# cmaestre/pcl_tracking

Measured on AMD Instinct MI355X. Metric: particles x input-points / sec per frame (tracked frames/sec @8192 particles per GPU), higher is better.
Workload: dtype f32

## Files before the change

### pcl_tracking_amd/csrc/pft_api.hip

```cpp
#include <math.h>
#include <stdio.h>
#include <string.h>

#include <stdlib.h>

#include <algorithm>
#include <cmath>
#include <string>
#include <vector>

#include "pft_internal.h"
#include "../../include/pft_segment.h"

#define HIPCHK(t, call)                                                                       \
  do {                                                                                        \
    hipError_t e_ = (call);                                                                   \
    if (e_ != hipSuccess) {                                                                   \
      (t)->err = std::string(#call) + ": " + hipGetErrorString(e_);                           \
      return PFT_ERR_HIP;                                                                     \
    }                                                                                         \
  } while (0)

struct EvPair {
  hipEvent_t a, b;
// ... 508 lines not shown
  if (debug) {
    HIPCHK(t, dalloc(&n.b.mark, cap));
    HIPCHK(t, dalloc(&n.pts, cap));
  }
  n.b.cap = cap;
  n.b.tab_cap = tab;
  if (c.b.st) {
    HIPCHK(t, hipMemcpyAsync(n.b.st, c.b.st, sizeof(PftChangeState), hipMemcpyDeviceToDevice, t->stream));
    for (int k = 0; k < 2; k++) {
      HIPCHK(t, hipMemcpyAsync(n.b.set_key[k], c.b.set_key[k], (size_t)c.b.cap * 8u, hipMemcpyDeviceToDevice, t->stream));
      HIPCHK(t, hipMemcpyAsync(n.b.set_cnt[k], c.b.set_cnt[k], (size_t)c.b.cap * 4u, hipMemcpyDeviceToDevice, t->stream));
    }
    HIPCHK(t, hipStreamSynchronize(t->stream));
  } else {
    HIPCHK(t, hipMemsetAsync(n.b.st, 0, sizeof(PftChangeState), t->stream));
  }
  cd_free(c);
  c = n;
  return PFT_OK;
}

PftSwitches pft_read_switches() {
  auto on = [](const char* name) { return getenv(name) != nullptr; };
  auto is1 = [](const char* name) { const char* e = getenv(name); return e && e[0] == '1'; };
  PftSwitches w = {};
  w.graph = is1("PFT_GRAPH");
  if (const char* b = getenv("PFT_FORCE_BUILDER")) w.builder = !strcmp(b, "single") ? 1 : (!strcmp(b, "sorted") ? 2 : 0);
  w.leaf_indirect = on("PFT_LEAF_INDIRECT") ? (int)is1("PFT_LEAF_INDIRECT") : -1;
  w.aabb_full = on("PFT_AABB_FULL");
  w.resample_one_lane = on("PFT_RESAMPLE_ONE_LANE");
  w.split_resample = on("PFT_SPLIT_RESAMPLE") || w.resample_one_lane;
  w.crop_two_pass = on("PFT_CROP_TWO_PASS");
  w.generic_descent = is1("PFT_GENERIC_DESCENT");
  w.ancestor_table = !on("PFT_ANCESTOR_TABLE") || is1("PFT_ANCESTOR_TABLE");
  w.exact_path = on("PFT_EXACT_SHELLS_ONLY") ? PftExactPath::shells : on("PFT_EXACT_PER_QUERY") ? PftExactPath::per_query : PftExactPath::sorted;
#ifdef PFT_DIAG
  if (const char* a = getenv("PFT_ABLATE")) w.ablate = atoi(a);
  w.skip_octree = on("PFT_DEBUG_SKIP_OCTREE");
#endif
  return w;
}

#ifdef PFT_DIAG
extern "C" void pft_debug_set_ablate(pft_tracker* t, int mask) { if (t) t->sw.ablate = mask; }
#endif

extern "C" int pft_create(const pft_config* cfg, pft_tracker** out) {
  if (!cfg || !out) return PFT_ERR_INVALID_ARG;
  *out = nullptr;
  if (cfg->abi_version != PFT_ABI_VERSION || cfg->particle_num <= 0 || cfg->iteration_num <= 0 ||
      cfg->world_size <= 0 || cfg->rank < 0 || cfg->rank >= cfg->world_size || cfg->use_normal != 0 ||
      cfg->particle_num % cfg->world_size != 0 || !(cfg->octree_resolution > 0) ||
      (cfg->sum_order != PFT_SUM_TREE && cfg->sum_order != PFT_SUM_PCL))
    return PFT_ERR_INVALID_ARG;
  if (cfg->particle_num > PFT_MAX_PARTICLES) return PFT_ERR_CAPACITY;
  if (cfg->kld_adaptive) {
    if (cfg->world_size != 1 || cfg->maximum_particle_num <= 0 || !(cfg->kld_epsilon > 0)) return PFT_ERR_INVALID_ARG;
    for (int k = 0; k < 6; k++)
      if (!(cfg->kld_bin_size[k] > 0)) return PFT_ERR_INVALID_ARG;
    if (cfg->maximum_particle_num >= PFT_POPM_MIN || cfg->particle_num >= PFT_POPM_MIN) return PFT_ERR_CAPACITY;
  }
  int ndev = 0;
  if (hipGetDeviceCount(&ndev) != hipSuccess || ndev <= 0 || cfg->device_id >= ndev) return PFT_ERR_NO_DEVICE;
  if (hipSetDevice(cfg->device_id) != hipSuccess) return PFT_ERR_NO_DEVICE;
  hipDeviceProp_t prop;
  if (hipGetDeviceProperties(&prop, cfg->device_id) != hipSuccess) return PFT_ERR_NO_DEVICE;

// ... 59 lines not shown
  A(dalloc(&t->d_jump, (size_t)1 << (3 * PFT_JUMP_MAX_LEVEL)));
  if (t->sw.ancestor_table) A(dalloc(&t->d_anc, PFT_ANC_CAP));
  A(dalloc(&t->d_alias_list, 2 * Pt));
  A(dalloc(&t->d_alias_pref, 2 * Pt));
  A(dalloc(&t->d_pop_part, (size_t)PFT_POPM_MAX_WGS * 16));
  A(dalloc(&t->d_alias_pos, Pt));
  A(dalloc(&t->d_raw_w, Pt));
  if (cfg->exact_nearest) {
    A(dalloc(&t->d_eg_start, (size_t)PFT_EG_CAP + 1));
    A(dalloc(&t->d_eg_cnt, (size_t)PFT_EG_CAP));
    A(dalloc(&t->d_eg_tile, (size_t)PFT_EG_CAP / 2048 + 2));
    A(dalloc(&t->d_ec_slot, (size_t)PFT_EG_CAP));
    A(dalloc(&t->d_ec_cells, (size_t)PFT_EC_SLOTS));
    A(dalloc(&t->d_ec_count, (size_t)PFT_EC_SLOTS));
    A(dalloc(&t->d_ec_base, (size_t)PFT_EC_SLOTS));
    t->ec_pool_cap = PFT_EC_POOL_MIN;
    A(dalloc(&t->d_ec_list, (size_t)t->ec_pool_cap));
    A(dalloc(&t->d_eq_cellq, (size_t)PFT_EG_CAP));
    A(dalloc(&t->d_eq_nq, (size_t)PFT_EC_SLOTS));
    A(dalloc(&t->d_eq_qbase, (size_t)PFT_EC_SLOTS));
    A(dalloc(&t->d_eq_bbase, (size_t)PFT_EC_SLOTS));
    A(dalloc(&t->d_eq_fill, (size_t)PFT_EC_SLOTS));
  }
  if (p.kld) {
    A(dalloc(&t->d_kld_table, (size_t)6 * p.kld_max + 128));
    A(dalloc(&t->d_kld_bins, (size_t)6 * p.kld_max));
  }
  A(hipHostMalloc(reinterpret_cast<void**>(&t->h_stat), 8 * sizeof(uint32_t), hipHostMallocMapped));
  if (t->h_stat) for (int i = 0; i < 8; i++) t->h_stat[i] = 0;
  A(dalloc(&t->d_hdr, 1));
  A(dalloc(&t->d_dbg_hdr, 1));
  if (e == hipSuccess) e = hipMemsetAsync(t->d_hdr, 0, sizeof(PftHeader), t->stream);
  if (e == hipSuccess) e = hipMemsetAsync(t->d_dbg_hdr, 0, sizeof(PftHeader), t->stream);
  if (e != hipSuccess) {
    pft_destroy(t);
    return PFT_ERR_HIP;
  }
  if (cfg->max_input_points) {
    int r = ensure_input_capacity(t, cfg->max_input_points);
    if (r != PFT_OK) {
      pft_destroy(t);
      return r;
    }
  }
  sync_dev(t);
  *out = t;
  return PFT_OK;
}

static void release_borrow(pft_tracker* t) {
  PftBorrow* b = t->borrow;
  t->borrow = nullptr;
  if (!b) return;
  b->tracker_alive = false;
  b->armed = false;
  if (!b->filter_alive) {
    hipEventDestroy(b->ev);
    delete b;
  }
}

extern "C" void pft_destroy(pft_tracker* t) {
  if (!t) return;
  if (t->stream) hipStreamSynchronize(t->stream);
  release_borrow(t);
  dfree(t->d_n_in);
// ... 2049 lines not shown
```

### pcl_tracking_amd/csrc/pft_device_utils.h

```cpp
#pragma once
#include <float.h>
#include <math.h>

#include "pft_internal.h"

#define WAVE 64
#define UNROLL_FENCE(j, every) do { if (((j) % (every)) == (every) - 1) __builtin_amdgcn_sched_barrier(0); } while (0)

__device__ __forceinline__ bool pft_unchanged(const uint32_t* gate) { return gate && *gate == 0u; }

__device__ __forceinline__ int lane_id() { return threadIdx.x & (WAVE - 1); }
__device__ __forceinline__ int wave_id() { return threadIdx.x >> 6; }

template <typename T>
__device__ __forceinline__ T wave_sum(T v) {
#pragma unroll
  for (int o = 32; o > 0; o >>= 1) v += __shfl_xor(v, o);
  return v;
}
template <int CTRL, int ROW_MASK>
__device__ __forceinline__ double dpp_move_f64(double v) {
  const unsigned long long b = (unsigned long long)__double_as_longlong(v);
  const int lo = __builtin_amdgcn_update_dpp(0, (int)(uint32_t)b, CTRL, ROW_MASK, 0xf, false);
  const int hi = __builtin_amdgcn_update_dpp(0, (int)(uint32_t)(b >> 32), CTRL, ROW_MASK, 0xf, false);
// ... 161 lines not shown
  float A = (float)cos((double)q.yaw), B = (float)sin((double)q.yaw);
  float C = (float)cos((double)q.pitch), D = (float)sin((double)q.pitch);
  float E = (float)cos((double)q.roll), F = (float)sin((double)q.roll);
  float DE = D * E, DF = D * F;
  m[0] = A * C;  m[1] = A * DF - B * E;  m[2] = B * F + A * DE;  m[3] = q.x;
  m[4] = B * C;  m[5] = A * E + B * DF;  m[6] = B * DE - A * F;  m[7] = q.y;
  m[8] = -D;     m[9] = C * F;           m[10] = C * E;          m[11] = q.z;
}

__device__ __forceinline__ void store_matrix(float* mats, uint32_t i, const float* m) {
  float4* dst = reinterpret_cast<float4*>(mats + 12 * (size_t)i);
  dst[0] = make_float4(m[0], m[1], m[2], m[3]);
  dst[1] = make_float4(m[4], m[5], m[6], m[7]);
  dst[2] = make_float4(m[8], m[9], m[10], m[11]);
}

__device__ __forceinline__ void load_matrix(const float* mats, uint32_t i, float* T) {
  const float4* tp = reinterpret_cast<const float4*>(mats + 12 * (size_t)i);
  float4 r0 = tp[0], r1 = tp[1], r2 = tp[2];
  T[0] = r0.x; T[1] = r0.y; T[2] = r0.z; T[3] = r0.w;
  T[4] = r1.x; T[5] = r1.y; T[6] = r1.z; T[7] = r1.w;
  T[8] = r2.x; T[9] = r2.y; T[10] = r2.z; T[11] = r2.w;
}

__device__ __forceinline__ void xform(const float* T, float x, float y, float z, float& ox, float& oy, float& oz) {
  ox = T[0] * x + T[1] * y + T[2] * z + T[3];
  oy = T[4] * x + T[5] * y + T[6] * z + T[7];
  oz = T[8] * x + T[9] * y + T[10] * z + T[11];
}

#include "pft_alias.h"

__device__ inline void pft_anc_window(PftHeader* hdr, const PftDev& d, int D, bool on, const double mn[3], double res) {
  const int L = D - PFT_ANC_UP;
  on = on && d.anc != nullptr && L >= 1;
  const float inv = (float)(1.0 / res);
  uint32_t lo[3] = {0u, 0u, 0u}, bits[3] = {0u, 0u, 0u};
  for (int a = 0; a < 3 && on; a++) {
    const float om = (float)mn[a];
    const float f0 = fmaxf(floorf((hdr->bbox[2 * a] - om) * inv), 0.0f);
    const float f1 = fmaxf(floorf((hdr->bbox[2 * a + 1] - om) * inv), 0.0f);
    const uint32_t top = (1u << L) - 1u;
    const uint32_t c0 = min(f0 < 2147483648.0f ? (uint32_t)f0 >> PFT_ANC_UP : top, top);
    const uint32_t c1 = min(f1 < 2147483648.0f ? (uint32_t)f1 >> PFT_ANC_UP : top, top);
    on = c1 >= c0;
    const uint32_t n = c1 - c0 + 1u;
    bits[a] = n > 1u ? 32u - (uint32_t)__clz((int)(n - 1u)) : 0u;
    lo[a] = min(c0, (1u << L) - (1u << bits[a]));
  }
  on = on && bits[0] + bits[1] + bits[2] <= PFT_ANC_CAP_BITS;
  hdr->anc_level = on ? L : 0;
  for (int a = 0; a < 3; a++) {
    hdr->anc_lo[a] = on ? lo[a] : 0u;
    hdr->anc_bits[a] = on ? bits[a] : 0u;
  }
  hdr->build_epoch = hdr->build_epoch + 1u;
}
```

### pcl_tracking_amd/csrc/pft_internal.h

```cpp
#pragma once
#include <hip/hip_runtime.h>
#include <stdint.h>

#include <vector>

#include "../../include/pft.h"

#define PFT_MAX_DEVICES 64
#define PFT_MAX_DEPTH 30
#define PFT_TABLE_MAX_DEPTH 10
#define PFT_MAX_GROW 40
#define PFT_JUMP_MAX_LEVEL 4
#ifndef PFT_ANC_CAP_BITS
#define PFT_ANC_CAP_BITS 18
#endif
#define PFT_ANC_CAP (1u << PFT_ANC_CAP_BITS)
#ifndef PFT_ANC_UP
#define PFT_ANC_UP 2
#endif
#define PFT_REF_CHUNK 256
#ifndef PFT_BUILD_THREADS
#define PFT_BUILD_THREADS 1024
#endif
#ifndef PFT_LIK_GROUPS
#define PFT_LIK_GROUPS 64
#endif
#ifndef PFT_LIK_CTR_STRIDE
#define PFT_LIK_CTR_STRIDE 16u
#endif
#ifndef PFT_LIK_THREADS
#define PFT_LIK_THREADS 1024
#endif
#ifndef PFT_LIK_WGS_PER_CU
#define PFT_LIK_WGS_PER_CU 2
#endif
#define PFT_POP_THREADS 1024
#define PFT_SORTED_BUILD_MIN 18000
#define PFT_EG_CAP (1u << 21)
#define PFT_EC_SLOTS (1u << 19)
#define PFT_EC_POOL (1u << 24)
#define PFT_EC_POOL_MIN (1u << 20)
#define PFT_POPM_THREADS 256
#define PFT_POPM_ITEMS 16
#define PFT_POPM_MAX_WGS 256
#define PFT_POPM_MIN (16 * PFT_POP_THREADS + 1)
#define PFT_MAX_PARTICLES (PFT_POPM_MAX_WGS * PFT_POPM_THREADS * PFT_POPM_ITEMS)

struct PftParams {
  double alpha;
  double maxd2;
  double res;
  double dist_w, hsv_w;
// ... 6 lines not shown
  uint32_t M_box;
  uint32_t ref_chunk;
  uint32_t split_last;
  uint32_t kld;
  uint32_t kld_max;
  double kld_z;
  double kld_eps;
  float kld_bin[6];
  double motion_ratio;
  int32_t sum_order;
};

struct PftHeader {
  float bbox[6];
  uint32_t n_crop;
  uint32_t error;
  double omin[3], omax[3];
  int32_t depth;
  int32_t use_table;
  uint32_t n_words;
  uint32_t n_leaves;
  uint32_t leaf_start;
  uint32_t lvl_start[PFT_MAX_DEPTH + 3];
  int32_t n_grow;
  int32_t build_path;
  uint32_t build_variant;
  int32_t leaf_indirect;
  int32_t jump_level;
  float margin_cells;
  float ominf[3];
  float inv_res;
  int32_t anc_level;
  uint32_t anc_lo[3], anc_bits[3];
  uint32_t build_epoch;
  uint32_t anc_epoch;
  uint32_t grow_idx[PFT_MAX_GROW];
  uint32_t grow_shift[PFT_MAX_GROW];
  uint32_t grow_old_depth[PFT_MAX_GROW];
  double grow_min[PFT_MAX_GROW + 1][3];
  double fit_ratio;
  pft_particle rep;
  pft_particle motion;
  uint32_t alias_m, alias_nh;
  float eg_g, eg_inv_g, eg_min[3];
  int32_t eg_dim[3];
  uint32_t eg_ncells;
  uint32_t p_active;
  uint32_t kld_k;
  unsigned long long stat_queries, stat_scanned;
  unsigned long long dbg[32];
  unsigned long long ticks[32];
  alignas(128) uint32_t lik_ctr[PFT_LIK_GROUPS * PFT_LIK_CTR_STRIDE];
  alignas(128) uint32_t ec_nslots;
  uint32_t ec_pool_used;
  unsigned long long eq_totals;
  alignas(128) uint32_t crop_ticket;
  uint32_t pop_bar[4];
  unsigned long long dbg_hard[5];
  uint32_t lik_layout[4];
};

struct PftDev {
  const float4* ref_xyz;
  const float4* ref_hsv;
  const float4* ref_box;
  const float4* in_pts;
// ... 101 lines not shown
  size_t n_in;
  int device_id;
  hipEvent_t done;
};
int pftf_view(pft_filter* f, PftFilterView* v);
void pftf_attach(pft_filter* f, PftBorrow* b);

void pftk_remove_zero_points(hipStream_t s, const pft_point_xyzrgba* in, uint32_t n, float4* xyz, uint8_t* flag,
                             uint32_t* tile, uint32_t* keep_idx, float4* keep_xyz, uint32_t* n_keep);
struct pft_segment;
int pftsg_device_id(const pft_segment* s);
struct pft_model;
struct PftModelView {
  const pft_point_xyzrgba* recentred;
  size_t n_recentred;
  const pft_point_xyzrgba* reference;
  size_t n_reference;
  float trans[16];
  uint32_t first_nonfinite;
  int device_id;
};
int pftm_view(const pft_model* m, PftModelView* v);

enum class PftExactPath { sorted, per_query, shells };
struct PftSwitches {
  bool graph;
  int builder;
  int leaf_indirect;
  bool aabb_full;
  bool split_resample;
  bool resample_one_lane;
  bool crop_two_pass;
  bool generic_descent;
  bool ancestor_table;
  PftExactPath exact_path;
  int ablate;
  bool skip_octree;
};
PftSwitches pft_read_switches();

void pftk_report(hipStream_t s, const pft_point_xyzrgba* pts, uint32_t n, const PftHeader* hdr, int sum_order,
                 pft_point_xyzrgba* tracked, pft_object_report* out);
void pftk_match(hipStream_t s, const PftParams& p, const PftDev& d, double min_ratio, uint32_t lost_after,
                pft_match_stats* out, int32_t* input_idx, float* sq_dist);
uint32_t pftk_spread_blocks(uint32_t n_max);
void pftk_spread(hipStream_t s, const PftDev& d, uint32_t n_max, double* part, uint32_t* part_zero, float* part_wmax,
                 uint32_t* part_imax, double max_pos_sigma, double min_n_eff, uint32_t after, pft_population_stats* out);
struct PftRqLattice {
  uint32_t n[3];
  float base[3], span[3];
};
struct PftRqScores {
  uint32_t *n_inliers, *n_matched;
  double *coherence, *sum_sq_dist, *inlier_sq_dist;
};
void pftk_reacquire_centroids(hipStream_t s, const pft_point_xyzrgba* pts, const uint32_t* first, const uint32_t* count,
                              uint32_t n_clusters, float* centres);
void pftk_reacquire_candidates(hipStream_t s, const float* centres, uint32_t K, const PftRqLattice& lat, pft_particle* part,
                               float* mats);
void pftk_reacquire_score(hipStream_t s, const PftParams& p, const PftDev& d, uint32_t K, double inlier_d2,
                          const PftRqScores& out);
void pftk_reacquire_select(hipStream_t s, const PftParams& p, const PftDev& d, const PftRqScores& sc, uint32_t K,
                           uint32_t n_centres, uint32_t per_centre, double accept_ratio, pft_reacquire_result* out);
struct PftRefineCtl;
struct PftRefineDev {
  PftRefineCtl* ctl;
  double* part;
// ... 59 lines not shown
```

### pcl_tracking_amd/csrc/pft_likelihood.hip

```cpp
#include "pft_device_utils.h"

#ifndef PFT_LIK_PENALTY
#define PFT_LIK_PENALTY 1
#endif

struct LikCtx {
  const uint32_t* words;
  const float* tab;
  uint32_t per_axis;
  const float* lut_h;
  const float* lut_s;
  const float* pen;
  const uint16_t* jump;
  int J;
  uint32_t lvlJ_start;
  const uint32_t* anc;
  uint32_t alo, abits;
  float margin, near_thr, ominx, ominy, ominz, inv_res, ncell;
  uint32_t leaf0;
  const uint16_t* leaf16;
};

struct HybridWords {
  const __attribute__((address_space(3))) uint32_t* lds;
  const uint32_t* __restrict__ glob;
  uint32_t n_lds;
  __device__ __forceinline__ uint32_t operator[](uint32_t i) const { return i < n_lds ? lds[i] : glob[i]; }
};

__device__ __forceinline__ double rcp_nr(double x) {
  double r = __builtin_amdgcn_rcp(x);
  double e = fma(-x, r, 1.0);
  r = fma(r, e, r);
  e = fma(-x, r, 1.0);
  r = fma(r, e, r);
  return r;
}

__device__ __forceinline__ bool face_violation(uint32_t kx, uint32_t ky, uint32_t kz, uint32_t lowf, uint32_t highf,
                                               int sh) {
  const uint32_t mx = (1u << sh) - 1u;
  const uint32_t rx = kx & mx, ry = ky & mx, rz = kz & mx;
  bool v = ((lowf & 1u) && rx == 0) || ((highf & 1u) && rx == mx);
  v |= ((lowf & 2u) && ry == 0) || ((highf & 2u) && ry == mx);
  v |= ((lowf & 4u) && rz == 0) || ((highf & 4u) && rz == mx);
  return v;
}

__device__ __forceinline__ int near_face_level(uint32_t k, bool low, bool high) {
  const uint32_t t = low ? k : ~k;
  const uint32_t c = min((uint32_t)(t == 0u ? -1 : __builtin_ctz(t)), 31u);
  return (low | high) ? (int)c : -1;
}

template <bool USE_TAB, bool FAST, bool DEBUG_NN, int LEAF, bool INDIRECT, typename WordPtr>
__device__ __forceinline__ void likelihood_items(const PftParams& prm, const PftDev& d, const LikCtx& cx, WordPtr W,
                                                 uint32_t n_particles, int D, uint32_t n_crop,
                                                 const double omin[3], int abl) {
  const int lane = lane_id(), w = wave_id(), nw = blockDim.x >> 6;
  const uint32_t M = prm.M, nchunk = prm.nchunk;
  const uint32_t G = min((uint32_t)PFT_LIK_GROUPS, gridDim.x), grp = blockIdx.x % G;
  const uint32_t gq = gridDim.x / G, gr = gridDim.x % G;
  const uint32_t wgs_in_grp = gq + (grp < gr ? 1u : 0u), waves_in_grp = wgs_in_grp * (uint32_t)nw;
  const uint32_t wgs_before = grp * gq + min(grp, gr);
  const uint32_t pb = (uint32_t)((unsigned long long)n_particles * wgs_before / gridDim.x);
  const uint32_t pe = (uint32_t)((unsigned long long)n_particles * (wgs_before + wgs_in_grp) / gridDim.x);
  const uint32_t np_grp = pe - pb, nbig = prm.split_last ? nchunk - prm.split_last : nchunk, nsmall = nchunk - nbig;
  const uint32_t small_len = prm.split_last ? prm.ref_chunk / prm.split_last : 0u;
  const uint32_t it_begin = 0u, it_end = np_grp * nchunk, big_items = np_grp * nbig;
  const uint32_t lw = (blockIdx.x / G) * (uint32_t)nw + (uint32_t)w;
  uint32_t* ctr = &d.hdr->lik_ctr[grp * PFT_LIK_CTR_STRIDE];
  const double res = prm.res;
  const double maxd2 = prm.maxd2;
  const double wd = prm.dist_w, whsv = prm.hsv_w;
  const float hw = prm.h_w, sw = prm.s_w, vw = prm.v_w;
  for (uint32_t item_v = it_begin + lw; item_v < it_end;) {
    const uint32_t item = (uint32_t)__builtin_amdgcn_readfirstlane((int)item_v);
    uint32_t pi, ch, cstart, clen;
    if (item < big_items) {
      pi = pb + item / nbig;
      ch = item % nbig;
      cstart = ch * prm.ref_chunk;
      clen = prm.ref_chunk;
    } else {
      const uint32_t r = item - big_items;
      pi = pb + r / nsmall;
      ch = nbig + r % nsmall;
      cstart = nbig * prm.ref_chunk + (r % nsmall) * small_len;
// ... 12 lines not shown
      float qx, qy, qz;
      xform(T, r.x, r.y, r.z, qx, qy, qz);
      if (n_crop == 0) {
        if (DEBUG_NN) {
          const size_t o = (size_t)pi * M + d.ref_perm[j];
          d.nn_idx[o] = -1;
          d.nn_d2[o] = INFINITY;
        }
        continue;
      }
      uint32_t node = 0, jx = 1, jy = 1, jz = 1;
      int lvl = 0;
      int dbg_fast = 0, dbg_gen = 0, dbg_jump = 0, dbg_hard = 0;
      if (FAST) {
        const float tx = (qx - cx.ominx) * cx.inv_res, ty = (qy - cx.ominy) * cx.inv_res,
                    tz = (qz - cx.ominz) * cx.inv_res;
        const float flx = floorf(tx), fly = floorf(ty), flz = floorf(tz);
        const bool inside = (int)(fminf(fminf(tx, ty), tz) >= 0.0f) & (int)(fmaxf(fmaxf(tx, ty), tz) < cx.ncell);
        const float fx = tx - flx, fy = ty - fly, fz = tz - flz;
        const float mg = cx.margin, mh = 1.0f - cx.margin;
        const uint32_t kx = inside ? (uint32_t)flx : 0u, ky = inside ? (uint32_t)fly : 0u,
                       kz = inside ? (uint32_t)flz : 0u;
        int V = -1;
        const float off = fmaxf(fmaxf(fabsf(fx - 0.5f), fabsf(fy - 0.5f)), fabsf(fz - 0.5f));
        if (__builtin_amdgcn_ballot_w64(off > cx.near_thr)) {
          const int vx = near_face_level(kx, fx < mg, fx > mh), vy = near_face_level(ky, fy < mg, fy > mh),
                    vz = near_face_level(kz, fz < mg, fz > mh);
          V = max(vx, max(vy, vz));
        }
        V = inside ? V : 31;
        int lim = min(D, D - 1 - V);
        bool inw = false;
        uint32_t ae = 0u;
        if (!INDIRECT && LEAF == 1 && cx.anc) {
          const uint32_t bx = cx.abits & 0xffu, by = (cx.abits >> 8) & 0xffu, bz = cx.abits >> 16;
          const uint32_t ux = (kx >> PFT_ANC_UP) - (cx.alo & 1023u), uy = (ky >> PFT_ANC_UP) - ((cx.alo >> 10) & 1023u),
                         uz = (kz >> PFT_ANC_UP) - (cx.alo >> 20);
          inw = ((ux >> bx) | (uy >> by) | (uz >> bz)) == 0u;
          ae = cx.anc[inw ? ux | (uy << bx) | (uz << (bx + by)) : 0u];
        }
        const int a = (int)(ae >> 27);
        const bool hit = inw & (a <= lim);
        node = hit ? (ae & 0x7ffffffu) : 0u;
        lvl = hit ? a : 0;
        lim = (hit & (a < D - PFT_ANC_UP)) ? a : lim;
        if (cx.J > 0 && __builtin_amdgcn_ballot_w64(!hit)) {
          const int sh = D - cx.J;
          const uint32_t e = cx.jump[(kx >> sh) | ((ky >> sh) << cx.J) | ((kz >> sh) << (2 * cx.J))];
          const bool take = !hit & (cx.J <= lim) & (e != 0u);
          node = take ? cx.lvlJ_start + e - 1u : node;
          lvl = take ? cx.J : lvl;
          if (DEBUG_NN) dbg_jump = take ? 1 : 0;
        }
        while (lvl < lim) {
          const int sh = D - lvl - 1;
          const uint32_t c = (((kx >> sh) & 1u) << 2) | (((ky >> sh) & 1u) << 1) | ((kz >> sh) & 1u);
          const uint32_t wv = W[node];
          if (!((wv >> c) & 1u)) break;
          node = (wv >> 8) + __popc(wv & 0xffu & ((1u << c) - 1u));
          lvl++;
          dbg_fast++;
        }
        const int up = D - lvl;
        const uint32_t top = 1u << lvl;
        jx = (kx >> up) | top; jy = (ky >> up) | top; jz = (kz >> up) | top;
      }
      if ((abl & 1) && lvl < D) {
        node = cx.leaf0;
        lvl = D;
      }
      for (; lvl < D; lvl++) {
        dbg_gen++;
        const uint32_t wv = W[node];
        const uint32_t mask = wv & 0xffu, base = wv >> 8;
        float cx0, cx1, cy0, cy1, cz0, cz1;
        if (USE_TAB) {
          const float2 tx2 = *reinterpret_cast<const float2*>(cx.tab - 2 + 2u * jx);
          const float2 ty2 = *reinterpret_cast<const float2*>(cx.tab + cx.per_axis - 2 + 2u * jy);
// ... 153 lines not shown
          hd2 = fabsf(1.0f + rh.x - th);
        else
          hd2 = fabsf(1.0f + th - rh.x);
        float h_diff;
        if (hd1 < hd2)
          h_diff = hw * hd1 * hd1;
        else
          h_diff = hw * hd2 * hd2;
        const float s_diff = sw * (rh.y - ts) * (rh.y - ts);
        const float v_diff = vw * (rh.z - tv) * (rh.z - tv);
        const float diff2 = h_diff + s_diff + v_diff;
        double Bq = 1.0 + whsv * (double)diff2;
        val += rcp_nr(A * Bq);
      }
    }
    val = wave_sum_lane63(val);
    if (lane == 63) d.partial[(size_t)pi * nchunk + ch] = val;
    {
      uint32_t nx = 0;
      if (lane == 0) nx = it_begin + waves_in_grp + atomicAdd(ctr, 1u);
      item_v = (uint32_t)__shfl((int)nx, 0);
    }
    if (DEBUG_NN) {
      st_q = wave_sum(st_q);
      st_s = wave_sum(st_s);
      if (lane == 0 && st_q) {
        atomicAdd(&d.hdr->stat_queries, st_q);
        atomicAdd(&d.hdr->stat_scanned, st_s);
      }
    }
  }
}

#define PFT_LIK_RUN(UT, FA, LF) likelihood_items<UT, FA, DEBUG_NN, LF, INDIRECT>(prm, d, cx, W, n_particles, D, n_crop, omin, abl)

template <bool DEBUG_NN, bool INDIRECT, bool GATED>
__global__ __launch_bounds__(PFT_LIK_THREADS, DEBUG_NN ? 1 : (PFT_LIK_THREADS * PFT_LIK_WGS_PER_CU) / 256) void k_likelihood(PftParams prm, PftDev d, uint32_t n_particles,
                                                                uint32_t lds_bytes, int flags) {
  const int allow_fast = flags & 1;
#ifdef PFT_DIAG
  const int abl = flags >> 8;
#else
  constexpr int abl = 0;
#endif
  extern __shared__ __attribute__((aligned(16))) unsigned char smem[];
  const PftHeader* hdr = d.hdr;
  if (GATED && pft_unchanged(d.gate)) return;
  if (d.p_active) n_particles = *d.p_active;
  const int D = hdr->depth;
  const uint32_t n_crop = (hdr->error || D <= 0 || (hdr->leaf_indirect != 0) != INDIRECT) ? 0u : hdr->n_crop;
  if (hdr->error && blockIdx.x == 0 && threadIdx.x == 0 && d.host_stat) {
    d.host_stat[2] = hdr->error;
    d.host_stat[3] |= hdr->error;
  }
  const uint32_t n_words = hdr->n_words;
  const int use_tab = hdr->use_table;
  const double omin[3] = {hdr->omin[0], hdr->omin[1], hdr->omin[2]};
  const uint32_t per_axis = use_tab ? (2u << D) : 0u;
  const bool fast = allow_fast && use_tab && hdr->margin_cells < 0.5f;
  int J = fast ? hdr->jump_level : 0;

  float* pen = reinterpret_cast<float*>(smem);
  constexpr uint32_t pen_bytes = PFT_LIK_PENALTY ? 256u * 8u * 4u : 0u;
  float* lut_h = reinterpret_cast<float*>(smem + pen_bytes);
  float* lut_s = lut_h + 256;
  float* tab = lut_s + 256;
  uint32_t used = pen_bytes + 2048u + 3u * per_axis * 4u;
// ... 56 lines not shown
      for (uint32_t i = threadIdx.x; i <= n_leaves; i += blockDim.x) lleaf[i] = (uint16_t)d.words[leaf_start + i];
  } else {
    for (uint32_t i = threadIdx.x; i < n_lds_words; i += blockDim.x) lwords[i] = d.words[i];
  }
  __syncthreads();

  LikCtx cx;
  cx.words = nullptr;
  cx.tab = tab;
  cx.per_axis = per_axis;
  cx.lut_h = lut_h;
  cx.lut_s = lut_s;
  cx.pen = pen;
  cx.jump = ljump;
  cx.J = J;
  cx.lvlJ_start = J > 0 ? hdr->lvl_start[J] : 0u;
  const bool anc_on = fast && (flags & 2) && d.anc && hdr->anc_level > 0 && hdr->anc_epoch == hdr->build_epoch;
  cx.anc = anc_on ? d.anc : nullptr;
  static_assert(PFT_TABLE_MAX_DEPTH <= 10, "ancestor table window coordinates are packed in 10 bits");
  cx.alo = hdr->anc_lo[0] | (hdr->anc_lo[1] << 10) | (hdr->anc_lo[2] << 20);
  cx.abits = hdr->anc_bits[0] | (hdr->anc_bits[1] << 8) | (hdr->anc_bits[2] << 16);
  cx.margin = hdr->margin_cells;
  cx.near_thr = 0.5f - 1.01f * hdr->margin_cells - 1.0e-6f;
  cx.ominx = hdr->ominf[0];
  cx.ominy = hdr->ominf[1];
  cx.ominz = hdr->ominf[2];
  cx.inv_res = hdr->inv_res;
  cx.ncell = (float)(1u << (D > 0 ? D : 0));
  cx.leaf0 = hdr->leaf_start;
  cx.leaf16 = lleaf;
  if (branch_only) {
    const uint32_t* W = lwords;
    if (fast)
      PFT_LIK_RUN(true, true, 2);
    else
      PFT_LIK_RUN(true, false, 2);
  } else if (words_in_lds && leaf16) {
    const uint32_t* W = lwords;
    if (fast)
      PFT_LIK_RUN(true, true, 1);
    else if (use_tab)
      PFT_LIK_RUN(true, false, 1);
    else
      PFT_LIK_RUN(false, false, 1);
  } else if (words_in_lds) {
    const uint32_t* W = lwords;
    if (fast)
      PFT_LIK_RUN(true, true, 0);
    else if (use_tab)
      PFT_LIK_RUN(true, false, 0);
    else
      PFT_LIK_RUN(false, false, 0);
  } else {
    HybridWords W;
    W.lds = (const __attribute__((address_space(3))) uint32_t*)lwords;
    W.glob = d.words;
    W.n_lds = n_lds_words;
    if (fast)
      PFT_LIK_RUN(true, true, 0);
    else if (use_tab)
      PFT_LIK_RUN(true, false, 0);
    else
      PFT_LIK_RUN(false, false, 0);
  }
}

extern "C" int pft_debug_likelihood_occupancy(void) {
  int nb = -1;
  uint32_t lds = ((uint32_t)pftk_max_lds_bytes() / (uint32_t)PFT_LIK_WGS_PER_CU) & ~255u;
  hipFuncSetAttribute(reinterpret_cast<const void*>(&k_likelihood<false, false, false>), hipFuncAttributeMaxDynamicSharedMemorySize, (int)lds);
  if (hipOccupancyMaxActiveBlocksPerMultiprocessor(&nb, reinterpret_cast<const void*>(&k_likelihood<false, false, false>), PFT_LIK_THREADS, lds) != hipSuccess) return -1;
  return nb;
}

void pftk_likelihood(hipStream_t s, const PftParams& p, const PftDev& d, uint32_t n_particles, bool debug_nn,
                     int num_cus, bool leaf_indirect, int flags) {
  static bool attr_set[PFT_MAX_DEVICES];
  uint32_t lds = ((uint32_t)pftk_max_lds_bytes() / (uint32_t)PFT_LIK_WGS_PER_CU) & ~255u;
  const int dev = pftk_cur_device();
  if (!attr_set[dev]) {
    const void* fns[8] = {
        reinterpret_cast<const void*>(&k_likelihood<false, false, false>), reinterpret_cast<const void*>(&k_likelihood<true, false, false>),
        reinterpret_cast<const void*>(&k_likelihood<false, true, false>), reinterpret_cast<const void*>(&k_likelihood<true, true, false>),
        reinterpret_cast<const void*>(&k_likelihood<false, false, true>), reinterpret_cast<const void*>(&k_likelihood<true, false, true>),
        reinterpret_cast<const void*>(&k_likelihood<false, true, true>), reinterpret_cast<const void*>(&k_likelihood<true, true, true>)};
    bool ok = true;
    for (int k = 0; k < 8; k++) ok = hipFuncSetAttribute(fns[k], hipFuncAttributeMaxDynamicSharedMemorySize, (int)lds) == hipSuccess && ok;
    attr_set[dev] = ok;
  }
  uint32_t items = n_particles * p.nchunk;
  uint32_t grid = (uint32_t)PFT_LIK_WGS_PER_CU * (uint32_t)num_cus;
  uint32_t need = (items + (PFT_LIK_THREADS / 64) - 1) / (PFT_LIK_THREADS / 64);
  if (need == 0) need = 1;
  if (grid > need) grid = need;
#define PFT_LIK_LAUNCH(DN, IND)                                                                                          \
  do {                                                                                                                   \
// ... 18 lines not shown
```

### pcl_tracking_amd/csrc/pft_octree.hip

```cpp
#include "pft_device_utils.h"

#ifdef PFT_DIAG
#define STAMP(k) do { if (threadIdx.x == 0) d.hdr->ticks[k] = wall_clock64(); } while (0)
#define TICK_NOW() wall_clock64()
#else
#define STAMP(k) do { } while (0)
#define TICK_NOW() 0ull
#endif

#include "pft_octree_box.h"

#define PFT_REPLAY_HEAD 1024u
__device__ __forceinline__ void box_replay(BuildSh& S, const float4* __restrict__ pts, uint32_t n, double res, unsigned long long* hdr_ticks) {
  const uint32_t tid = threadIdx.x, nt = blockDim.x;
  const uint32_t head = n < PFT_REPLAY_HEAD ? n : PFT_REPLAY_HEAD;
  float lmn[3] = {FLT_MAX, FLT_MAX, FLT_MAX}, lmx[3] = {-FLT_MAX, -FLT_MAX, -FLT_MAX};
  const uint32_t wt = tid - WAVE, ws = nt - WAVE;
  auto local_aabb = [&]() {
    for (uint32_t i0 = PFT_REPLAY_HEAD + wt; i0 < n; i0 += 8u * ws) {
      float4 q[8];
#pragma unroll
      for (uint32_t k = 0; k < 8u; k++) q[k] = pts[min(i0 + k * ws, n - 1u)];
#pragma unroll
      for (uint32_t k = 0; k < 8u; k++) {
// ... 535 lines not shown
    const uint32_t lds_total = lds_bytes / 4u, var = S.variant;
    const bool tried = lds_total - ((size_t)n * 5u / 2u + 64u <= lds_total ? ((n + 3u) & ~3u) : 0u) >= 64u;
    hdr->build_variant = var | ((var && !(var & 8u) && tried) ? 32u : 0u) | ((ok && use_table && S.jump > 0) ? 64u : 0u) |
                         (rescue ? 128u : 0u) | ((uint32_t)copy_leaf_pts << 8);
    hdr->leaf_indirect = copy_leaf_pts == 2 ? 1 : 0;
    if (d.host_stat) d.host_stat[1] = (uint32_t)D;
    hdr->jump_level = (ok && use_table) ? S.jump : 0;
    hdr->n_leaves = ok ? n_leaves : 0;
    hdr->leaf_start = ok ? leaf_start : 0;
    hdr->n_words = ok ? leaf_start + n_leaves + 1 : 0;
  }
  if (tid == 64) {
    double maxabs = 0.0;
    for (int a = 0; a < 3; a++) maxabs = fmax(maxabs, fmax(fabs(S.mn[a]), fabs(S.mx[a])));
    const double eta = maxabs * 1.1920928955078125e-07;
    const double s_top = prm.res * (double)(1u << (D > 0 ? D - 1 : 0));
    const double E = 9.0 * eta + 40.0 * 5.9604644775390625e-08 * s_top;
    double mc = 2.0 * E / prm.res + 1.0e-3;
    hdr->margin_cells = (float)(mc < 0.25 ? mc : 1.0);
  }
  if (tid == 128) hdr->inv_res = (float)(1.0 / prm.res);
  if (tid == 320) pft_anc_window(hdr, d, D, ok && use_table && copy_leaf_pts == 0, S.mn, prm.res);
  if (tid >= 192 && tid < 195) {
    const int a = (int)tid - 192;
    hdr->ominf[a] = (float)S.mn[a];
    hdr->omin[a] = n > 0 ? S.mn[a] : 0.0;
    hdr->omax[a] = n > 0 ? S.mx[a] : 0.0;
  }
  if (tid >= 256 && tid < 256 + PFT_MAX_DEPTH + 3 && (int)tid - 256 <= D + 1) hdr->lvl_start[tid - 256] = S.lvl[tid - 256];
}

__device__ __forceinline__ void anc_fill(const PftDev& d, uint32_t gid, uint32_t stride) {
  const PftHeader* hdr = d.hdr;
  const int L = hdr->anc_level;
  if (L <= 0) return;
  const uint32_t bx = hdr->anc_bits[0], by = hdr->anc_bits[1], n = 1u << (bx + by + hdr->anc_bits[2]);
  const uint32_t x0 = hdr->anc_lo[0], y0 = hdr->anc_lo[1], z0 = hdr->anc_lo[2];
  const int J = hdr->jump_level <= L ? hdr->jump_level : 0;
  const uint32_t lvlJ = J > 0 ? hdr->lvl_start[J] : 0u;
  for (uint32_t c = gid; c < n; c += stride) {
    const uint32_t x = x0 + (c & ((1u << bx) - 1u)), y = y0 + ((c >> bx) & ((1u << by) - 1u)), z = z0 + (c >> (bx + by));
    uint32_t node = 0;
    int lvl = 0;
    if (J > 0) {
      const int sh = L - J;
      const uint32_t e = d.jump[(x >> sh) | ((y >> sh) << J) | ((z >> sh) << (2 * J))];
      node = e ? lvlJ + e - 1u : 0u;
      lvl = e ? J : 0;
    }
    for (; lvl < L; lvl++) {
      const int sh = L - lvl - 1;
      const uint32_t ch = (((x >> sh) & 1u) << 2) | (((y >> sh) & 1u) << 1) | ((z >> sh) & 1u);
      const uint32_t wv = d.words[node];
      if (!((wv >> ch) & 1u)) break;
      node = (wv >> 8) + __popc(wv & 0xffu & ((1u << ch) - 1u));
    }
    d.anc[c] = ((uint32_t)lvl << 27) | node;
  }
  if (gid == 0) d.hdr->anc_epoch = hdr->build_epoch;
}

template <bool GATED>
__global__ __launch_bounds__(256) void k_leaf_gather(PftDev d) {
  if (GATED && pft_unchanged(d.gate)) return;
  const PftHeader* hdr = d.hdr;
  const uint32_t pos = blockIdx.x * 256u + threadIdx.x;
  if (hdr->error || hdr->depth <= 0) return;
  if (pos < hdr->n_crop) d.leaf_pts[pos] = d.crop_pts[d.leaf_order[pos]];
  anc_fill(d, pos, gridDim.x * 256u);
}

#ifndef PFT_OCTREE_GATED_TU
extern template __global__ void k_octree_build<true>(PftParams, PftDev, uint32_t, int, int);
extern template __global__ void k_leaf_gather<true>(PftDev);

static void pftk_octree_set_attr() {
  static bool attr_set[PFT_MAX_DEVICES];
  const uint32_t lds = ((uint32_t)pftk_max_lds_bytes() - 10240u) & ~15u;
  const int dev = pftk_cur_device();
  if (!attr_set[dev])
    attr_set[dev] = hipFuncSetAttribute(reinterpret_cast<const void*>(&k_octree_build<false>),
                                        hipFuncAttributeMaxDynamicSharedMemorySize, (int)lds) == hipSuccess &&
                    hipFuncSetAttribute(reinterpret_cast<const void*>(&k_octree_build<true>),
                                        hipFuncAttributeMaxDynamicSharedMemorySize, (int)lds) == hipSuccess;
}

void pftk_octree(hipStream_t s, const PftParams& p, const PftDev& d, uint32_t expected_points, bool indirect) {
  const uint32_t lds = ((uint32_t)pftk_max_lds_bytes() - 10240u) & ~15u;
  pftk_octree_set_attr();
  const int mode = indirect ? 2 : (expected_points <= 5000u ? 1 : 0);
// ... 20 lines not shown
```

Before: 835.3 billion.

## Adaptively choose ancestor-table level, preferring one level above leaves

The ancestor lookup table is now built at depth D-1 when the crop bounding box fits the table cap, and falls back to D-2 otherwise, instead of always using D-2. A finer table lets more likelihood queries start their octree descent closer to the leaf, skipping descent steps. The table fill is also reworked to walk parents at D-2 and expand each into its eight children in one pass. This adds a template specialization for the shift amount, a new header field, and the risk of larger table fills or more window misses when the box is large.

```diff
diff --git a/pcl_tracking_amd/csrc/pft_api.hip b/pcl_tracking_amd/csrc/pft_api.hip
--- a/pcl_tracking_amd/csrc/pft_api.hip
+++ b/pcl_tracking_amd/csrc/pft_api.hip
@@ -564,7 +564,8 @@
   w.split_resample = on("PFT_SPLIT_RESAMPLE") || w.resample_one_lane;
   w.crop_two_pass = on("PFT_CROP_TWO_PASS");
   w.generic_descent = is1("PFT_GENERIC_DESCENT");
-  w.ancestor_table = !on("PFT_ANCESTOR_TABLE") || is1("PFT_ANCESTOR_TABLE");
+  w.ancestor_table = 3;
+  if (const char* a = getenv("PFT_ANCESTOR_TABLE")) w.ancestor_table = a[0] == '1' ? 1 : a[0] == '2' ? 2 : !strcmp(a, "auto") ? 3 : 0;
   w.exact_path = on("PFT_EXACT_SHELLS_ONLY") ? PftExactPath::shells : on("PFT_EXACT_PER_QUERY") ? PftExactPath::per_query : PftExactPath::sorted;
 #ifdef PFT_DIAG
   if (const char* a = getenv("PFT_ABLATE")) w.ablate = atoi(a);
@@ -690,6 +691,10 @@
   A(dalloc(&t->d_dbg_hdr, 1));
   if (e == hipSuccess) e = hipMemsetAsync(t->d_hdr, 0, sizeof(PftHeader), t->stream);
   if (e == hipSuccess) e = hipMemsetAsync(t->d_dbg_hdr, 0, sizeof(PftHeader), t->stream);
+  static_assert(offsetof(PftHeader, anc_up) % 4 == 0, "set with a 32-bit fill");
+  if (e == hipSuccess)
+    e = hipMemsetD32Async(reinterpret_cast<hipDeviceptr_t>(&t->d_hdr->anc_up),
+                          t->sw.ancestor_table == 1 ? PFT_ANC_UP_MAX : PFT_ANC_UP_MIN, 1, t->stream);
   if (e != hipSuccess) {
     pft_destroy(t);
     return PFT_ERR_HIP;
diff --git a/pcl_tracking_amd/csrc/pft_device_utils.h b/pcl_tracking_amd/csrc/pft_device_utils.h
--- a/pcl_tracking_amd/csrc/pft_device_utils.h
+++ b/pcl_tracking_amd/csrc/pft_device_utils.h
@@ -217,27 +217,34 @@
 #include "pft_alias.h"
 
 __device__ inline void pft_anc_window(PftHeader* hdr, const PftDev& d, int D, bool on, const double mn[3], double res) {
-  const int L = D - PFT_ANC_UP;
-  on = on && d.anc != nullptr && L >= 1;
+  on = on && d.anc != nullptr;
   const float inv = (float)(1.0 / res);
+  float f0[3], f1[3];
+  for (int a = 0; a < 3; a++) {
+    const float om = (float)mn[a];
+    f0[a] = fmaxf(floorf((hdr->bbox[2 * a] - om) * inv), 0.0f);
+    f1[a] = fmaxf(floorf((hdr->bbox[2 * a + 1] - om) * inv), 0.0f);
+  }
+  int L = 0;
   uint32_t lo[3] = {0u, 0u, 0u}, bits[3] = {0u, 0u, 0u};
-  for (int a = 0; a < 3 && on; a++) {
-    const float om = (float)mn[a];
-    const float f0 = fmaxf(floorf((hdr->bbox[2 * a] - om) * inv), 0.0f);
-    const float f1 = fmaxf(floorf((hdr->bbox[2 * a + 1] - om) * inv), 0.0f);
-    const uint32_t top = (1u << L) - 1u;
-    const uint32_t c0 = min(f0 < 2147483648.0f ? (uint32_t)f0 >> PFT_ANC_UP : top, top);
-    const uint32_t c1 = min(f1 < 2147483648.0f ? (uint32_t)f1 >> PFT_ANC_UP : top, top);
-    on = c1 >= c0;
-    const uint32_t n = c1 - c0 + 1u;
-    bits[a] = n > 1u ? 32u - (uint32_t)__clz((int)(n - 1u)) : 0u;
-    lo[a] = min(c0, (1u << L) - (1u << bits[a]));
-  }
-  on = on && bits[0] + bits[1] + bits[2] <= PFT_ANC_CAP_BITS;
-  hdr->anc_level = on ? L : 0;
+  for (int up = hdr->anc_up < PFT_ANC_UP_MIN ? PFT_ANC_UP_MIN : hdr->anc_up; on && L == 0 && up <= PFT_ANC_UP_MAX && D - up >= 1; up++) {
+    const int l = D - up;
+    bool fits = true;
+    for (int a = 0; a < 3 && fits; a++) {
+      const uint32_t top = (1u << l) - 1u;
+      const uint32_t c0 = min(f0[a] < 2147483648.0f ? (uint32_t)f0[a] >> up : top, top);
+      const uint32_t c1 = min(f1[a] < 2147483648.0f ? (uint32_t)f1[a] >> up : top, top);
+      fits = c1 >= c0;
+      const uint32_t n = c1 - c0 + 1u;
+      bits[a] = n > 1u ? 32u - (uint32_t)__clz((int)(n - 1u)) : 0u;
+      lo[a] = min(c0, (1u << l) - (1u << bits[a]));
+    }
+    if (fits && bits[0] + bits[1] + bits[2] <= PFT_ANC_CAP_BITS) L = l;
+  }
+  hdr->anc_level = L;
   for (int a = 0; a < 3; a++) {
-    hdr->anc_lo[a] = on ? lo[a] : 0u;
-    hdr->anc_bits[a] = on ? bits[a] : 0u;
+    hdr->anc_lo[a] = L > 0 ? lo[a] : 0u;
+    hdr->anc_bits[a] = L > 0 ? bits[a] : 0u;
   }
   hdr->build_epoch = hdr->build_epoch + 1u;
 }
diff --git a/pcl_tracking_amd/csrc/pft_internal.h b/pcl_tracking_amd/csrc/pft_internal.h
--- a/pcl_tracking_amd/csrc/pft_internal.h
+++ b/pcl_tracking_amd/csrc/pft_internal.h
@@ -15,9 +15,8 @@
 #define PFT_ANC_CAP_BITS 18
 #endif
 #define PFT_ANC_CAP (1u << PFT_ANC_CAP_BITS)
-#ifndef PFT_ANC_UP
-#define PFT_ANC_UP 2
-#endif
+#define PFT_ANC_UP_MIN 1
+#define PFT_ANC_UP_MAX 2
 #define PFT_REF_CHUNK 256
 #ifndef PFT_BUILD_THREADS
 #define PFT_BUILD_THREADS 1024
@@ -90,6 +89,7 @@
   float inv_res;
   int32_t anc_level;
   uint32_t anc_lo[3], anc_bits[3];
+  int32_t anc_up;
   uint32_t build_epoch;
   uint32_t anc_epoch;
   uint32_t grow_idx[PFT_MAX_GROW];
@@ -257,7 +257,7 @@
   bool resample_one_lane;
   bool crop_two_pass;
   bool generic_descent;
-  bool ancestor_table;
+  int ancestor_table;
   PftExactPath exact_path;
   int ablate;
   bool skip_octree;
diff --git a/pcl_tracking_amd/csrc/pft_likelihood.hip b/pcl_tracking_amd/csrc/pft_likelihood.hip
--- a/pcl_tracking_amd/csrc/pft_likelihood.hip
+++ b/pcl_tracking_amd/csrc/pft_likelihood.hip
@@ -53,7 +53,7 @@
   return (low | high) ? (int)c : -1;
 }
 
-template <bool USE_TAB, bool FAST, bool DEBUG_NN, int LEAF, bool INDIRECT, typename WordPtr>
+template <bool USE_TAB, bool FAST, bool DEBUG_NN, int LEAF, bool INDIRECT, int UP, typename WordPtr>
 __device__ __forceinline__ void likelihood_items(const PftParams& prm, const PftDev& d, const LikCtx& cx, WordPtr W,
                                                  uint32_t n_particles, int D, uint32_t n_crop,
                                                  const double omin[3], int abl) {
@@ -132,10 +132,10 @@
         int lim = min(D, D - 1 - V);
         bool inw = false;
         uint32_t ae = 0u;
-        if (!INDIRECT && LEAF == 1 && cx.anc) {
+        if (UP > 0 && cx.anc) {
           const uint32_t bx = cx.abits & 0xffu, by = (cx.abits >> 8) & 0xffu, bz = cx.abits >> 16;
-          const uint32_t ux = (kx >> PFT_ANC_UP) - (cx.alo & 1023u), uy = (ky >> PFT_ANC_UP) - ((cx.alo >> 10) & 1023u),
-                         uz = (kz >> PFT_ANC_UP) - (cx.alo >> 20);
+          const uint32_t ux = (kx >> UP) - (cx.alo & 1023u), uy = (ky >> UP) - ((cx.alo >> 10) & 1023u),
+                         uz = (kz >> UP) - (cx.alo >> 20);
           inw = ((ux >> bx) | (uy >> by) | (uz >> bz)) == 0u;
           ae = cx.anc[inw ? ux | (uy << bx) | (uz << (bx + by)) : 0u];
         }
@@ -143,7 +143,7 @@
         const bool hit = inw & (a <= lim);
         node = hit ? (ae & 0x7ffffffu) : 0u;
         lvl = hit ? a : 0;
-        lim = (hit & (a < D - PFT_ANC_UP)) ? a : lim;
+        lim = (hit & (a < D - UP)) ? a : lim;
         if (cx.J > 0 && __builtin_amdgcn_ballot_w64(!hit)) {
           const int sh = D - cx.J;
           const uint32_t e = cx.jump[(kx >> sh) | ((ky >> sh) << cx.J) | ((kz >> sh) << (2 * cx.J))];
@@ -363,7 +363,7 @@
   }
 }
 
-#define PFT_LIK_RUN(UT, FA, LF) likelihood_items<UT, FA, DEBUG_NN, LF, INDIRECT>(prm, d, cx, W, n_particles, D, n_crop, omin, abl)
+#define PFT_LIK_RUN(UT, FA, LF, UP) likelihood_items<UT, FA, DEBUG_NN, LF, INDIRECT, UP>(prm, d, cx, W, n_particles, D, n_crop, omin, abl)
 
 template <bool DEBUG_NN, bool INDIRECT, bool GATED>
 __global__ __launch_bounds__(PFT_LIK_THREADS, DEBUG_NN ? 1 : (PFT_LIK_THREADS * PFT_LIK_WGS_PER_CU) / 256) void k_likelihood(PftParams prm, PftDev d, uint32_t n_particles,
@@ -486,36 +486,38 @@
   if (branch_only) {
     const uint32_t* W = lwords;
     if (fast)
-      PFT_LIK_RUN(true, true, 2);
+      PFT_LIK_RUN(true, true, 2, 0);
     else
-      PFT_LIK_RUN(true, false, 2);
+      PFT_LIK_RUN(true, false, 2, 0);
   } else if (words_in_lds && leaf16) {
     const uint32_t* W = lwords;
-    if (fast)
-      PFT_LIK_RUN(true, true, 1);
+    if (fast && !INDIRECT && anc_on && D - hdr->anc_level == PFT_ANC_UP_MIN)
+      PFT_LIK_RUN(true, true, 1, PFT_ANC_UP_MIN);
+    else if (fast)
+      PFT_LIK_RUN(true, true, 1, INDIRECT ? 0 : PFT_ANC_UP_MAX);
     else if (use_tab)
-      PFT_LIK_RUN(true, false, 1);
+      PFT_LIK_RUN(true, false, 1, 0);
     else
-      PFT_LIK_RUN(false, false, 1);
+      PFT_LIK_RUN(false, false, 1, 0);
   } else if (words_in_lds) {
     const uint32_t* W = lwords;
     if (fast)
-      PFT_LIK_RUN(true, true, 0);
+      PFT_LIK_RUN(true, true, 0, 0);
     else if (use_tab)
-      PFT_LIK_RUN(true, false, 0);
+      PFT_LIK_RUN(true, false, 0, 0);
     else
-      PFT_LIK_RUN(false, false, 0);
+      PFT_LIK_RUN(false, false, 0, 0);
   } else {
     HybridWords W;
     W.lds = (const __attribute__((address_space(3))) uint32_t*)lwords;
     W.glob = d.words;
     W.n_lds = n_lds_words;
     if (fast)
-      PFT_LIK_RUN(true, true, 0);
+      PFT_LIK_RUN(true, true, 0, 0);
     else if (use_tab)
-      PFT_LIK_RUN(true, false, 0);
+      PFT_LIK_RUN(true, false, 0, 0);
     else
-      PFT_LIK_RUN(false, false, 0);
+      PFT_LIK_RUN(false, false, 0, 0);
   }
 }
 
diff --git a/pcl_tracking_amd/csrc/pft_octree.hip b/pcl_tracking_amd/csrc/pft_octree.hip
--- a/pcl_tracking_amd/csrc/pft_octree.hip
+++ b/pcl_tracking_amd/csrc/pft_octree.hip
@@ -591,30 +591,50 @@
 
 __device__ __forceinline__ void anc_fill(const PftDev& d, uint32_t gid, uint32_t stride) {
   const PftHeader* hdr = d.hdr;
-  const int L = hdr->anc_level;
+  const int L = hdr->anc_level, D = hdr->depth;
   if (L <= 0) return;
-  const uint32_t bx = hdr->anc_bits[0], by = hdr->anc_bits[1], n = 1u << (bx + by + hdr->anc_bits[2]);
+  const bool expand = L == D - 1;
+  const int P = expand ? L - 1 : L;
+  const uint32_t bx = hdr->anc_bits[0], by = hdr->anc_bits[1], bz = hdr->anc_bits[2];
   const uint32_t x0 = hdr->anc_lo[0], y0 = hdr->anc_lo[1], z0 = hdr->anc_lo[2];
-  const int J = hdr->jump_level <= L ? hdr->jump_level : 0;
+  const uint32_t px0 = expand ? x0 >> 1 : x0, py0 = expand ? y0 >> 1 : y0, pz0 = expand ? z0 >> 1 : z0;
+  const uint32_t nx = expand ? ((x0 + (1u << bx) - 1u) >> 1) - px0 + 1u : 1u << bx;
+  const uint32_t ny = expand ? ((y0 + (1u << by) - 1u) >> 1) - py0 + 1u : 1u << by;
+  const uint32_t nz = expand ? ((z0 + (1u << bz) - 1u) >> 1) - pz0 + 1u : 1u << bz;
+  const uint32_t n = nx * ny * nz;
+  const int J = hdr->jump_level <= P ? hdr->jump_level : 0;
   const uint32_t lvlJ = J > 0 ? hdr->lvl_start[J] : 0u;
   for (uint32_t c = gid; c < n; c += stride) {
-    const uint32_t x = x0 + (c & ((1u << bx) - 1u)), y = y0 + ((c >> bx) & ((1u << by) - 1u)), z = z0 + (c >> (bx + by));
+    const uint32_t cyz = c / nx;
+    const uint32_t x = px0 + (c - cyz * nx), y = py0 + cyz % ny, z = pz0 + cyz / ny;
     uint32_t node = 0;
     int lvl = 0;
     if (J > 0) {
-      const int sh = L - J;
+      const int sh = P - J;
       const uint32_t e = d.jump[(x >> sh) | ((y >> sh) << J) | ((z >> sh) << (2 * J))];
       node = e ? lvlJ + e - 1u : 0u;
       lvl = e ? J : 0;
     }
-    for (; lvl < L; lvl++) {
-      const int sh = L - lvl - 1;
+    for (; lvl < P; lvl++) {
+      const int sh = P - lvl - 1;
       const uint32_t ch = (((x >> sh) & 1u) << 2) | (((y >> sh) & 1u) << 1) | ((z >> sh) & 1u);
       const uint32_t wv = d.words[node];
       if (!((wv >> ch) & 1u)) break;
       node = (wv >> 8) + __popc(wv & 0xffu & ((1u << ch) - 1u));
     }
-    d.anc[c] = ((uint32_t)lvl << 27) | node;
+    const uint32_t e = ((uint32_t)lvl << 27) | node;
+    if (!expand) {
+      d.anc[c] = e;
+      continue;
+    }
+    const uint32_t wv = lvl == P ? d.words[node] : 0u;
+    const uint32_t mask = wv & 0xffu, base = wv >> 8;
+#pragma unroll
+    for (uint32_t ch = 0; ch < 8u; ch++) {
+      const uint32_t ux = 2u * x + (ch >> 2) - x0, uy = 2u * y + ((ch >> 1) & 1u) - y0, uz = 2u * z + (ch & 1u) - z0;
+      const uint32_t ec = (mask >> ch) & 1u ? ((uint32_t)L << 27) | (base + __popc(mask & ((1u << ch) - 1u))) : e;
+      if (((ux >> bx) | (uy >> by) | (uz >> bz)) == 0u) d.anc[ux | (uy << bx) | (uz << (bx + by))] = ec;
+    }
   }
   if (gid == 0) d.hdr->anc_epoch = hdr->build_epoch;
 }
```

Result: no change. 842.9 billion (median of 6 runs) (+0.9%).
